# cgisky1980/Qwen3-TTS-Rust

Measured on AMD Instinct MI355X. Metric: audio_sec_per_s, higher is better.
Workload: dtype bf16

## Files before the change

include/q3tts.h:

```cpp
#ifndef Q3TTS_H
#define Q3TTS_H

#include <stdint.h>

#ifdef __cplusplus
extern "C" {
#endif

#define Q3TTS_OK 0
#define Q3TTS_ERR_INVALID (-1)
#define Q3TTS_ERR_DEVICE (-2)
#define Q3TTS_ERR_OOM (-3)
#define Q3TTS_ERR_IO (-4)
#define Q3TTS_ERR_STATE (-5)
#define Q3TTS_ERR_UNSUPPORTED (-6)
#define Q3TTS_MAX_BATCH 256

#define Q3TTS_MAX_UPSAMPLE 4
#define Q3TTS_MAX_DEC_BLOCKS 8


typedef struct q3tts_model_config {
    int32_t t_n_layer, t_d_model, t_n_head, t_n_kv_head, t_head_dim, t_d_ffn, t_vocab;
    float t_rope_theta;
// ... 272 lines not shown
                    int32_t* n_samples_out);
int q3tts_k_vocoder_latent(q3tts_engine* e, const int32_t* codes, int32_t n_frames, int32_t chunk_frames, float* out);
typedef struct q3tts_voc_tap {
    char name[32];
    int32_t dtype, layout, hist_rows, rows, channels, reserved;
    uint64_t offset;
} q3tts_voc_tap;
int q3tts_k_vocoder_taps(q3tts_engine* e, const int32_t* codes, int32_t n_frames, int32_t chunk_frames, int32_t tap_call, void* buf,
                         uint64_t buf_bytes, q3tts_voc_tap* recs, int32_t rec_cap, int32_t* n_recs);
int q3tts_k_vocoder_bench(q3tts_engine* e, int32_t n_slots, int32_t chunks, float* ms_per_chunk);
int q3tts_k_gguf_read(const char* path, const char* tensor, float* out, int64_t cap, int64_t* nelem, int64_t* dims4, int32_t* ggml_type);
int q3tts_k_gguf_meta(const char* path, const char* key, int32_t* value_type, int32_t* elem_type, int64_t* count, double* values,
                      int64_t values_cap, char* str, int64_t str_cap, int64_t* str_bytes);
int q3tts_k_probe(q3tts_engine* e, int32_t enable);
int q3tts_k_mfma_bf16(int32_t device, const uint16_t* a, const uint16_t* b, const float* c, float* d, int32_t n_cases, int32_t chain);
int q3tts_k_bgemm(int32_t device, const uint16_t* xb, int32_t B, int32_t K, const uint16_t* w_bf16, int32_t N, const float* ssp, int32_t ntiles,
                  int32_t d_norm, float eps, int32_t epilogue, const float* nw_next, float* y, uint16_t* yb, float* ssp_out, uint64_t* keys,
                  int32_t iters, float* mean_kernel_ms);
int q3tts_k_bgemm_policy(int32_t big);
int q3tts_k_attend_policy(int32_t decode, int32_t prefill);
int q3tts_k_pred_variant(q3tts_engine* e, int32_t force);
int q3tts_k_text_ready(int32_t n_text, int32_t closed, int32_t n_frames);
int q3tts_k_bgemm_pick(int32_t B, int32_t K, int32_t N, int32_t epilogue, int32_t w_once, int32_t q8, int32_t* out5);
int q3tts_k_bgemm_q8(int32_t device, const uint16_t* xb, int32_t B, int32_t K, const int8_t* q, const uint16_t* d_f16, int32_t N, const float* ssp,
                     int32_t ntiles, int32_t d_norm, float eps, int32_t epilogue, const float* nw_next, float* y, uint16_t* yb, float* ssp_out,
                     uint64_t* keys, int32_t iters, float* mean_kernel_ms);
int q3tts_k_bgemm_q8a8(int32_t device, const int8_t* aq, const float* ad, int32_t B, int32_t K, const int8_t* q, const uint16_t* d_f16, int32_t N,
                       const float* ssp, int32_t ntiles, int32_t d_norm, float eps, int32_t epilogue, const float* nw_next, float* y, int8_t* yq,
                       float* yd, float* ssp_out, int32_t iters, float* mean_kernel_ms);
int q3tts_k_bgemm_q8a8_argmax(int32_t device, const int8_t* aq, const float* ad, int32_t B, int32_t K, const int8_t* q, const uint16_t* d_f16, int32_t N,
                              const float* ssp, int32_t ntiles, int32_t d_norm, float eps, int32_t* ids_out);
int q3tts_k_bgemm_voc(int32_t device, const uint16_t* xb, int32_t B, int32_t K, const uint16_t* w_bf16, int32_t N, int32_t epilogue, const float* bias,
                      int32_t bias_n, const float* col_scale, int32_t seg_rows, int32_t gap_rows, float* y, uint16_t* yb, int32_t want_yb);
int q3tts_k_project(int32_t device, const float* x, int32_t rows, int32_t n_in, const float* w, const float* bias, int32_t n_out, const float* nw,
                    float* y, uint16_t* xb, float* ssp);
int q3tts_k_norm_inputs(int32_t device, const float* x, int32_t rows, int32_t d, const float* nw, uint16_t* xb, float* ssp);
int q3tts_k_alloc_upload(q3tts_engine* e, int64_t bytes, int64_t* mismatches);
int q3tts_k_pcm_pack(int32_t device, const float* src, int32_t rows, int64_t stride, const int32_t* ent_row, const int32_t* ent_first,
                     const int32_t* ent_count, const int64_t* ent_dst, int32_t n_ent, int32_t format, void* out, int64_t out_n);
int q3tts_k_resample_table(int32_t rate_in, int32_t rate_out, int32_t* L, int32_t* M, int32_t* H, float* tab, int64_t cap, int64_t* n);
int q3tts_k_pcm_resample(int32_t device, const float* src, int32_t rows, int64_t stride, const int32_t* row_len, const int32_t* row_final,
                         const int32_t* ent_row, const int32_t* ent_first, const int32_t* ent_count, const int64_t* ent_dst, int32_t n_ent,
                         int32_t rate_in, int32_t rate_out, int32_t format, void* out, int64_t out_n, int32_t iters, float* mean_ms);
int q3tts_k_row_buckets(int32_t max_batch, int32_t* out, int32_t cap);
int q3tts_k_bucket_steps(const q3tts_engine* e, int64_t* out, int32_t cap);
int q3tts_k_prefix_stats(const q3tts_engine* e, int64_t* out2);
// ... 9 lines not shown
```

qwen3-tts-rust_amd/csrc/q3_attend.hip:

```cpp
#include "q3_kernels.h"

__device__ __forceinline__ uint2 pack_bf16x4(float a, float b, float c, float d) {
    return make_uint2((uint32_t)q3_bf16(a) | ((uint32_t)q3_bf16(b) << 16), (uint32_t)q3_bf16(c) | ((uint32_t)q3_bf16(d) << 16));
}
__device__ __forceinline__ uint16_t* k_cache_elem(uint16_t* khead, int pos, int lane) {
    const int blk = pos >> 6, kl = pos & 63, c = lane >> 1, e0 = 4 * (lane & 1);
    return khead + ((size_t)(blk * (Q3_ATT_HD >> 3) + c) * 64 + kl) * 8 + e0;
}
__device__ __forceinline__ float prep_rinv(const float4 x4, float eps, int hd) {
    float acc = 0.0f;
    acc = fmaf(x4.x, x4.x, acc); acc = fmaf(x4.y, x4.y, acc); acc = fmaf(x4.z, x4.z, acc); acc = fmaf(x4.w, x4.w, acc);
    acc = wave_sum(acc);
    return 1.0f / sqrtf(acc / (float)hd + eps);
}
__device__ __forceinline__ void prep_norm(const float4 x4, float rinv, const float4 w4, float y[4]) {
    y[0] = (x4.x * rinv) * w4.x; y[1] = (x4.y * rinv) * w4.y; y[2] = (x4.z * rinv) * w4.z; y[3] = (x4.w * rinv) * w4.w;
}
__device__ __forceinline__ void prep_rope(const float y[4], const float4 c4, const float4 s4, int hl, int lane, float o[4]) {
    const float cc[4] = {c4.x, c4.y, c4.z, c4.w}, ss[4] = {s4.x, s4.y, s4.z, s4.w};
#pragma unroll
    for (int e = 0; e < 4; ++e) {
        const float other = __shfl_xor(y[e], hl);
        o[e] = (lane < hl) ? fmaf(-other, ss[e], y[e] * cc[e])
                           : fmaf(other, ss[e], y[e] * cc[e]);
// ... 190 lines not shown
    for (int e = 0; e < 8; ++e) {
        o[e] = o[e] + __shfl_xor(o[e], 16);
        o[e] = o[e] + __shfl_xor(o[e], 32);
    }
    if (kg == 0) {
#pragma unroll
        for (int e = 0; e < 8; ++e) ow[(hh * 4 + sw) * hd + dl * 8 + e] = o[e];
    }
    __syncthreads();
    Q3_STAMP(a, 3);
    for (int i = tid; i < R * hd; i += R * 256) {
        const int h2 = i / hd, d = i - h2 * hd;
        const float r0 = ow[(h2 * 4 + 0) * hd + d], r1 = ow[(h2 * 4 + 1) * hd + d], r2 = ow[(h2 * 4 + 2) * hd + d],
                    r3 = ow[(h2 * 4 + 3) * hd + d];
        const float ov = ((r0 + r1) + r2) + r3;
        const float l = ((lw[h2 * 4] + lw[h2 * 4 + 1]) + lw[h2 * 4 + 2]) + lw[h2 * 4 + 3];
        att_out1(a, row, g * R + h2, d, ov / l);
    }
#ifdef Q3_STAMPS
    Q3_STAMP(a, 4);
    asm volatile("s_waitcnt vmcnt(0)" ::: "memory");
    Q3_STAMP(a, 5);
#endif
}
__global__ __launch_bounds__(256, 2) void k_attend_gqa2(Q3Attend a) {
    extern __shared__ __attribute__((aligned(16))) float smem[];
    const int g = blockIdx.x, row = blockIdx.y;
    Q3_STAMP(a, 0);
    int pos, slot;
    q3_row_map(row, a.row_pos, a.row_slot, a.slot_mod, a.pos_const, &pos, &slot);
    if (pos < 0) return;
    constexpr int hd = Q3_ATT_HD, half = hd >> 1, nl = hd >> 2;
    const int T = pos + 1, Tcap = a.n_ctx;
    const int tid = threadIdx.x, sw = tid >> 6, lane = tid & 63, kg = lane >> 4, dl = lane & 15;
    float* p0 = smem;
    float* p1 = p0 + Tcap;
    float* qh = p1 + Tcap;
    float* ow = qh + 2 * hd;
    float* lw = ow + 2 * 4 * hd;
    float* mw = lw + 8;
    uint32_t* knew = (uint32_t*)(mw + 8);
    uint32_t* vnew = knew + 64;
    const Q3QkPrep& pr = a.prep;
    const size_t hb = ((size_t)slot * a.Hkv + g) * a.n_ctx;
    const uint16_t* kb = a.kc + hb * hd;
    const uint16_t* vb = a.vc + hb * hd;
// ... 14 lines not shown
            prep_norm(x4, prep_rinv(x4, pr.eps, hd), w4, y);
            const float cc[4] = {c4.x, c4.y, c4.z, c4.w}, ss[4] = {s4.x, s4.y, s4.z, s4.w};
            float o[4];
#pragma unroll
            for (int e = 0; e < 4; ++e) {
                const float other = __shfl_xor(y[e], 16);
                o[e] = (lane < 16) ? fmaf(-other, ss[e], y[e] * cc[e]) : fmaf(other, ss[e], y[e] * cc[e]);
            }
            if (lane < nl) {
                if (sw < 2) *(float4*)(qh + sw * hd + 4 * lane) = (float4){o[0], o[1], o[2], o[3]};
                else {
                    const uint2 kk = pack_bf16x4(o[0], o[1], o[2], o[3]);
                    *(uint2*)k_cache_elem(pr.kc + hb * hd, pos, lane) = kk;
                    *(uint2*)(knew + 2 * lane) = kk;
                }
            }
        } else if (lane < nl) {
            const uint2 vk = pack_bf16x4(x4.x, x4.y, x4.z, x4.w);
            *(uint2*)(pr.vc + (hb + pos) * hd + 4 * lane) = vk;
            *(uint2*)(vnew + 2 * lane) = vk;
        }
    }
    __builtin_amdgcn_sched_barrier(0);
    uint4 kv[16], vv[4][4];
    {
        const uint4* kp = (const uint4*)(kb + (size_t)min(sw, (T - 1) >> 6) * 64 * hd) + lane;
#pragma unroll
        for (int c = 0; c < 16; ++c) kv[c] = kp[c * 64];
#pragma unroll
        for (int tr = 0; tr < 2; ++tr)
#pragma unroll
            for (int u = 0; u < 4; ++u) vv[tr][u] = *(const uint4*)(vb + (size_t)min(64 * tr + 4 * sw + kg + 16 * u, T - 1) * hd + dl * 8);
    }
    __builtin_amdgcn_sched_barrier(0);
    Q3_LDS_BARRIER();
    Q3_STAMP(a, 1);
    const float scale = 1.0f / sqrtf((float)hd);
    float ml0 = -INFINITY, ml1 = -INFINITY;
    for (int blk = sw; blk * 64 < T; blk += 4) {
        const int t = blk * 64 + lane;
        if (blk != sw) {
            const uint4* kp = (const uint4*)(kb + (size_t)blk * 64 * hd) + lane;
#pragma unroll
            for (int c = 0; c < 16; ++c) kv[c] = kp[c * 64];
        }
        if (t == pos) {
#pragma unroll
            for (int c = 0; c < 16; ++c) kv[c] = *(const uint4*)(knew + 4 * c);
        }
        float s0 = 0.0f, s1 = 0.0f;
#pragma unroll
        for (int c = 0; c < 16; ++c) {
            const float4 qa = *(const float4*)(qh + c * 8), qb = *(const float4*)(qh + c * 8 + 4);
            const float4 ra = *(const float4*)(qh + hd + c * 8), rb = *(const float4*)(qh + hd + c * 8 + 4);
            s0 = att_dot8(qa, qb, kv[c], s0);
            s1 = att_dot8(ra, rb, kv[c], s1);
        }
        s0 = s0 * scale; s1 = s1 * scale;
        if (t < T) { p0[t] = s0; p1[t] = s1; ml0 = fmaxf(ml0, s0); ml1 = fmaxf(ml1, s1); }
    }
#pragma unroll
    for (int tr = 2; tr < 4; ++tr)
#pragma unroll
        for (int u = 0; u < 4; ++u) vv[tr][u] = *(const uint4*)(vb + (size_t)min(64 * tr + 4 * sw + kg + 16 * u, T - 1) * hd + dl * 8);
    ml0 = wave_max(ml0); ml1 = wave_max(ml1);
    if (lane == 0) { mw[sw] = ml0; mw[4 + sw] = ml1; }
    Q3_LDS_BARRIER();
    const float m0 = fmaxf(fmaxf(mw[0], mw[1]), fmaxf(mw[2], mw[3])), m1 = fmaxf(fmaxf(mw[4], mw[5]), fmaxf(mw[6], mw[7]));
    float ls0 = 0.0f, ls1 = 0.0f;
    for (int blk = sw; blk * 64 < T; blk += 4) {
        const int t = blk * 64 + lane;
        if (t < T) {
            const float e0 = q3_expf(p0[t] - m0), e1 = q3_expf(p1[t] - m1);
            p0[t] = e0; p1[t] = e1; ls0 += e0; ls1 += e1;
        }
    }
    ls0 = wave_sum(ls0); ls1 = wave_sum(ls1);
    if (lane == 0) { lw[sw] = ls0; lw[4 + sw] = ls1; }
    Q3_LDS_BARRIER();
    Q3_STAMP(a, 2);
    float o0[8], o1[8];
#pragma unroll
    for (int e = 0; e < 8; ++e) { o0[e] = 0.0f; o1[e] = 0.0f; }
    const uint4 vn = *(const uint4*)(vnew + 4 * dl);
#pragma unroll
    for (int tr = 0; tr < 4; ++tr) {
        const int t0 = 64 * tr + 4 * sw + kg;
        if (64 * tr >= T) break;
#pragma unroll
        for (int u = 0; u < 4; ++u) {
            const int t = t0 + 16 * u;
            if (t < T) {
                const float pa = p0[t], pb = p1[t];
                const uint4 w = (t == pos) ? vn : vv[tr][u];
                att_pv8x2(pa, pb, w, o0, o1);
            }
        }
    }
    for (int t0 = 256 + 4 * sw + kg; t0 < T; t0 += 64) {
        uint4 vl[4];
#pragma unroll
        for (int u = 0; u < 4; ++u) vl[u] = *(const uint4*)(vb + (size_t)min(t0 + 16 * u, T - 1) * hd + dl * 8);
#pragma unroll
        for (int u = 0; u < 4; ++u) {
            const int t = t0 + 16 * u;
            if (t < T) {
                const float pa = p0[t], pb = p1[t];
                const uint4 w = (t == pos) ? vn : vl[u];
                att_pv8x2(pa, pb, w, o0, o1);
            }
        }
    }
#pragma unroll
    for (int e = 0; e < 8; ++e) {
        o0[e] = o0[e] + __shfl_xor(o0[e], 16); o0[e] = o0[e] + __shfl_xor(o0[e], 32);
        o1[e] = o1[e] + __shfl_xor(o1[e], 16); o1[e] = o1[e] + __shfl_xor(o1[e], 32);
    }
    if (kg == 0) {
        *(float4*)(ow + (0 * 4 + sw) * hd + dl * 8) = (float4){o0[0], o0[1], o0[2], o0[3]}; *(float4*)(ow + (0 * 4 + sw) * hd + dl * 8 + 4) = (float4){o0[4], o0[5], o0[6], o0[7]};
        *(float4*)(ow + (1 * 4 + sw) * hd + dl * 8) = (float4){o1[0], o1[1], o1[2], o1[3]}; *(float4*)(ow + (1 * 4 + sw) * hd + dl * 8 + 4) = (float4){o1[4], o1[5], o1[6], o1[7]};
    }
    Q3_LDS_BARRIER();
    Q3_STAMP(a, 3);
    if (tid < 128) {
        const int h2 = tid >> 6, d0 = 2 * (tid & 63);
// ... 465 lines not shown
```

qwen3-tts-rust_amd/csrc/q3_bgemm.hip:

```cpp
#include "q3_kernels.h"

typedef __bf16 bf16x8 __attribute__((ext_vector_type(8)));
typedef uint32_t u32x4 __attribute__((ext_vector_type(4)));

__device__ __forceinline__ float bg_wave_sum(float v) {
#pragma unroll
    for (int m = 32; m >= 1; m >>= 1) v = v + __shfl_xor(v, m);
    return v;
}

__device__ __forceinline__ size_t bg_yoff(const Q3BGemm& g, int row) {
    return g.seg_rows ? (size_t)(row / g.seg_rows) * g.seg_stride + (size_t)(row % g.seg_rows) * g.ldy : (size_t)row * g.ldy;
}
__device__ __forceinline__ float bg_gelu_erf(float x) { return 0.5f * x * (1.0f + erff(x * 0.70710678118654752f)); }

__device__ __forceinline__ u32x4 bg_ldw(const u32x4* p, bool nt) { return nt ? __builtin_nontemporal_load(p) : *p; }

__device__ __forceinline__ bf16x8 bg_q8_frag(uint32_t lo, uint32_t hi) {
    union { u32x4 u; bf16x8 v; } r;
#define Q8F(w_, b_) __float_as_uint((float)(int)(signed char)((w_) >> (8 * (b_))))
    r.u.x = (Q8F(lo, 0) >> 16) | (Q8F(lo, 1) & 0xffff0000u); r.u.y = (Q8F(lo, 2) >> 16) | (Q8F(lo, 3) & 0xffff0000u);
    r.u.z = (Q8F(hi, 0) >> 16) | (Q8F(hi, 1) & 0xffff0000u); r.u.w = (Q8F(hi, 2) >> 16) | (Q8F(hi, 3) & 0xffff0000u);
#undef Q8F
    return r.v;
}
__device__ __forceinline__ float bg_f16(uint32_t bits) { return (float)__builtin_bit_cast(_Float16, (unsigned short)bits); }

#define BG_PH(RT_, NT_) ((8 * (RT_) * (NT_) > 64 && ((RT_) * (NT_)) % 2 == 0) ? 2 : 1)
template <int RT, int NT, int D, bool NTW, bool Q8>
__global__ __launch_bounds__(512) void k_bgemm(Q3BGemm g) {
    extern __shared__ float part[];
    __shared__ float srow[64];
    Q3_STAMP(g, 0);
    constexpr int TR = RT * NT * 4;
    const int wave = threadIdx.x >> 6, lane = threadIdx.x & 63, kq = lane >> 4, r = lane & 15;
    int cg = blockIdx.x, rc = blockIdx.y;
    if (gridDim.y > 1 && (gridDim.x & 7) == 0) {
        const int id = blockIdx.x + gridDim.x * blockIdx.y, G = gridDim.y;
        rc = (id >> 3) % G; cg = (id & 7) + (id / (8 * G)) * 8;
    }
    const int nb0 = cg * NT, row0 = rc * RT * 16, kblocks = g.K >> 5, per = g.K >> 8, kb0 = wave * per;
    const int B = g.B;
    const u32x4* ap[RT];
#pragma unroll
    for (int i = 0; i < RT; ++i) {
        const int R = g.a_row0 + min(row0 + 16 * i + r, B - 1);
        ap[i] = (const u32x4*)g.a + ((size_t)(R >> 4) * kblocks + kb0) * 64 + kq * 16 + (R & 15);
    }
    const u32x4* wp[NT];
#pragma unroll
    for (int j = 0; j < NT; ++j) wp[j] = (const u32x4*)g.w + ((size_t)(nb0 + j) * kblocks + kb0) * 64 + lane;
    constexpr int NR = 2 * RT;
// ... 374 lines not shown
                    if (g.nw_next) {
                        if (live) g.yb[q3_atile_off(row, col, g.N >> 5)] = q3_bf16(xv * g.nw_next[col]);
                        float sq = xv * xv;
                        sq = sq + __shfl_xor(sq, 1); sq = sq + __shfl_xor(sq, 2); sq = sq + __shfl_xor(sq, 4); sq = sq + __shfl_xor(sq, 8);
                        if (live && c == 0) g.ssp_out[(size_t)row * g.ld_ssp_out + tile] = sq;
                    }
                }
            }
        }
}
static bool bg_big_ok(const Q3BGemm& g) {
    return g.B >= 256 && !g.wscale && (g.epi == Q3_EPI_STORE || g.epi == Q3_EPI_RESID || g.epi == Q3_EPI_SWIGLU) && g.N % 128 == 0 && g.a_row0 % 16 == 0 &&
           !g.bias && !g.col_scale && !g.seg_rows && !(g.epi == Q3_EPI_RESID && g.yb && !g.nw_next);
}
static void bg_launch_big(const Q3BGemm& g, hipStream_t s) {
    const dim3 grid(g.N / 128, (g.B + 127) / 128);
    hipLaunchKernelGGL(k_bgemm_big, grid, dim3(256), BB_NS * 16384, s, g);
}

template <int RT, int NT>
struct BgInst {
    static constexpr int S = RT + NT;
    static constexpr int D = S <= 3 ? 8 : (S == 4 ? 5 : (S == 5 ? 4 : (S == 6 ? 3 : 2)));
    static constexpr size_t lds = (size_t)8 * RT * NT * 4 * 64 * 4 / BG_PH(RT, NT);
    static void prepare() {
        if (lds > 65536) {
            hipFuncSetAttribute((const void*)k_bgemm<RT, NT, D, false, false>, hipFuncAttributeMaxDynamicSharedMemorySize, (int)lds);
            hipFuncSetAttribute((const void*)k_bgemm<RT, NT, D, true, false>, hipFuncAttributeMaxDynamicSharedMemorySize, (int)lds);
            hipFuncSetAttribute((const void*)k_bgemm<RT, NT, D, false, true>, hipFuncAttributeMaxDynamicSharedMemorySize, (int)lds);
            hipFuncSetAttribute((const void*)k_bgemm<RT, NT, D, true, true>, hipFuncAttributeMaxDynamicSharedMemorySize, (int)lds);
        }
    }
    static void launch(const Q3BGemm& g, dim3 grid, hipStream_t s) {
        const bool nt = g.w_once && grid.y == 1;
        if (g.wscale) {
            if (nt) hipLaunchKernelGGL((k_bgemm<RT, NT, D, true, true>), grid, dim3(512), lds, s, g);
            else hipLaunchKernelGGL((k_bgemm<RT, NT, D, false, true>), grid, dim3(512), lds, s, g);
        } else if (nt) hipLaunchKernelGGL((k_bgemm<RT, NT, D, true, false>), grid, dim3(512), lds, s, g);
        else hipLaunchKernelGGL((k_bgemm<RT, NT, D, false, false>), grid, dim3(512), lds, s, g);
    }
};
#define BG_EACH(X) X(1, 1) X(1, 2) X(1, 3) X(2, 1) X(2, 2) X(2, 3) X(3, 1) X(3, 2) X(3, 3) X(4, 1) X(4, 2) X(4, 3)
static int g_lds_cap_kb = 0;
static int g_big_policy = 0;
void q3_bgemm_prepare() {
    static Q3PerDevice pd;
    static std::once_flag env_once;
    std::call_once(env_once, []() {
        const char* ev = getenv("Q3TTS_BG_BIG"); g_big_policy = ev ? atoi(ev) : 0;
        ev = getenv("Q3TTS_BG_LDS_CAP"); g_lds_cap_kb = ev ? atoi(ev) : 0;
    });
    pd.ensure(1, []() {
        hipFuncSetAttribute((const void*)k_bgemm_big, hipFuncAttributeMaxDynamicSharedMemorySize, BB_NS * 16384);
#define P(RT_, NT_) BgInst<RT_, NT_>::prepare();
        BG_EACH(P)
#undef P
    });
}

static int g_force_rt = 0, g_force_nt = 0;
void q3_bgemm_force(int rt, int nt) { g_force_rt = rt; g_force_nt = nt; }
void q3_bgemm_big_policy(int policy) { q3_bgemm_prepare(); g_big_policy = policy; }
// ... 14 lines not shown
            const bool mid = g.B > 64 && g.B <= 512 && !g.wscale;
            if (g.B > 64 && !mid && RT != 4 && !(RT == 2 && g.B <= 128)) continue;
            const long chunks = (g.B + 16 * RT - 1) / (16 * RT);
            if (g.B <= 64 && RT > 1 && 16 * (RT - 1) * chunks >= g.B) continue;
            const long wgs = (long)(tiles / NT) * chunks, rounds = (wgs + 255) / 256;
            const long cost = rounds * ((g.wscale ? 32L * RT + 17L * NT : 32L * (RT + NT)) * g.K + 24000L);
            const bool tie = mid ? (NT > bestNT || (NT == bestNT && wgs > bestWgs)) : (wgs > bestWgs || (wgs == bestWgs && NT > bestNT));
            if (bestCost < 0 || cost < bestCost || (cost == bestCost && tie)) { bestCost = cost; bestRT = RT; bestNT = NT; bestWgs = wgs; }
        }
    if (g_force_rt > 0 && g_force_nt > 0 && tiles % g_force_nt == 0) { bestRT = g_force_rt; bestNT = g_force_nt; }
    *rt = bestRT; *nt = bestNT;
}
void q3_bgemm_pick(const Q3BGemm& g, int* rt, int* nt, int* d, int* ntw, int* big) {
    q3_bgemm_prepare();
    bg_pick(g, rt, nt, big);
    *d = 0; *ntw = 0;
    if (*big) return;
#define X(RT_, NT_) if (*rt == RT_ && *nt == NT_) *d = BgInst<RT_, NT_>::D;
    BG_EACH(X)
#undef X
    *ntw = (g.w_once && (g.B + 16 * *rt - 1) / (16 * *rt) == 1) ? 1 : 0;
}

static int bg_check(const Q3BGemm& g) {
    if (g.B < 1 || g.N % 16 || g.K % 256 || g.K < 256 || !g.a || !g.w || g.a_row0 < 0) return -1;
    if (g.wscale && g.K % 512) return -1;
    if (g.yb && (((g.epi == Q3_EPI_RESID || g.epi == Q3_EPI_GELU) && g.N % 32) || (g.epi == Q3_EPI_SWIGLU && g.N % 64))) return -1;
    if ((g.epi == Q3_EPI_SWIGLU || g.epi == Q3_EPI_GELU) && (!g.yb)) return -1;
    if (g.bias && g.bias_n < 1) return -1;
    if (g.ssp && g.ntiles < 1) return -1;
    return 0;
}

int q3_launch_bgemm(const Q3BGemm& g, hipStream_t s) {
    if (bg_check(g)) return -1;
    q3_bgemm_prepare();
    int bestRT, bestNT, big;
    bg_pick(g, &bestRT, &bestNT, &big);
    if (big) { bg_launch_big(g, s); return 0; }
    const dim3 grid(g.N / 16 / bestNT, (g.B + 16 * bestRT - 1) / (16 * bestRT));
#define L(RT_, NT_) if (bestRT == RT_ && bestNT == NT_) { BgInst<RT_, NT_>::launch(g, grid, s); return 0; }
    BG_EACH(L)
#undef L
    return -1;
}

// ... 22 lines not shown
```

qwen3-tts-rust_amd/csrc/q3_hooks.hip:

```cpp
#include "q3_engine.h"

#include <cstdio>
#include <cstring>

#define TRY(x) do { int rc__ = (x); if (rc__ != Q3TTS_OK) return rc__; } while (0)
#define HK(call) do { hipError_t er__ = (call); if (er__ != hipSuccess) return q3_set_err(nullptr, Q3TTS_ERR_DEVICE, std::string(#call) + ": " + hipGetErrorString(er__)); } while (0)

struct DevBuf {
    void* p = nullptr;
    ~DevBuf() { if (p) hipFree(p); }
    template <class T> operator T*() const { return (T*)p; }
    int put(const void* host, size_t bytes) {
        if (hipMalloc(&p, bytes + 64) != hipSuccess || hipMemset(p, 0, bytes + 64) != hipSuccess) return q3_set_err(nullptr, Q3TTS_ERR_OOM, "hipMalloc");
        if (host) HK(hipMemcpy(p, host, bytes, hipMemcpyHostToDevice));
        return Q3TTS_OK;
    }
    int alloc(size_t bytes) { return put(nullptr, bytes); }
    int get(void* host, size_t bytes) const { HK(hipMemcpy(host, p, bytes, hipMemcpyDeviceToHost)); return Q3TTS_OK; }
};

template <class F>
static int time_launches(int iters, F launch, float* mean_ms) {
    if (iters <= 0 || !mean_ms) return Q3TTS_OK;
    hipEvent_t a, b; HK(hipEventCreate(&a)); HK(hipEventCreate(&b));
// ... 151 lines not shown
    qp.cs = dcs; qp.sn = dsn; qp.kc = dkc; qp.vc = dvc; qp.n_ctx = n_ctx; qp.row_pos = dpp; qp.row_slot = dps;
    if (npre && q3_launch_qk_prep(qp, nullptr)) return q3_set_err(nullptr, Q3TTS_ERR_INVALID, "attention decode hook: the q/k prep launch was refused");
    int old_dec = 0, old_pre = 0;
    q3_attend_policy_get(&old_dec, &old_pre);
    if (policy >= 0) q3_attend_policy(policy, old_pre);
    for (int pass = 0; pass < (out_bf16 ? 2 : 1); ++pass) {
        HK(hipMemcpy(dlast.p, last.data(), last.size() * 4, hipMemcpyHostToDevice));
        Q3QkPrep dq = qp; dq.qkv = dlast; dq.rows = n_slots; dq.row_pos = ddp; dq.row_slot = dds;
        Q3Attend at{}; at.qkv = dlast; at.ld = ld; at.rows = n_slots; at.ldo = nq; at.Hq = Hq; at.Hkv = Hkv; at.hd = hd;
        at.kc = dkc; at.vc = dvc; at.n_ctx = n_ctx; at.row_pos = dq.row_pos; at.row_slot = dq.row_slot;
        at.fused = 1; at.prep = dq;
        if (pass == 0) { at.out = dout; at.out_bf16 = 0; }
        else { at.out = dob; at.out_bf16 = 1; }
        if (q3_launch_attend(at, nullptr)) { q3_attend_policy(old_dec, old_pre); return q3_set_err(nullptr, Q3TTS_ERR_INVALID, "attention decode hook: the attention launch was refused"); }
        const hipError_t er = hipDeviceSynchronize();
        if (er != hipSuccess) { q3_attend_policy(old_dec, old_pre); return q3_set_err(nullptr, Q3TTS_ERR_DEVICE, std::string("attention decode hook: ") + hipGetErrorString(er)); }
    }
    q3_attend_policy(old_dec, old_pre);
    HK(hipGetLastError());
    TRY(dout.get(out_f32, (size_t)n_slots * nq * 4));
    return out_bf16 ? untile_host(dob, n_slots, nq, out_bf16) : Q3TTS_OK;
}

struct AttHook {
    int n_slots = 0, n_ctx = 0, Hq = 0, Hkv = 0, ld = 0, nq = 0, form = 0, out_rows = 0, rt16 = 0;
    DevBuf qn, kn, cs, sn, kc, vc, out, osc;
    static const char* check(const float* qkv, int n_slots, int n_ctx, int Hq, int Hkv, int hd, const float* qnw, const float* knw, int form, const void* out,
                             const float* out_scale) {
        if (!qkv || !qnw || !knw || !out) return "a null argument";
        if (hd != Q3_ATT_HD) return "head_dim must be 128";
        if (n_slots <= 0 || n_slots > 4096) return "1 .. 4096 slots";
        if (n_ctx <= 0 || n_ctx % 64 || n_ctx > 8192) return "n_ctx must be a multiple of 64 in 64 .. 8192";
        if (Hkv <= 0 || Hq <= 0 || Hq % Hkv || Hq > 64) return "n_head must be a multiple of n_kv_head";
        const int R = Hq / Hkv;
        if (R != 1 && R != 2 && R != 4) return "the GQA ratio must be 1, 2 or 4";
        if (form < 0 || form > 2) return "out_form 0 (f32), 1 (bf16) or 2 (Q8_0)";
        if (form == 2 && !out_scale) return "out_form 2 needs out_scale";
        return nullptr;
    }
    int init(int slots, int nctx, int hq, int hkv, const float* qnw, const float* knw, float theta, const int32_t* sections, int out_form, int rows) {
        n_slots = slots; n_ctx = nctx; Hq = hq; Hkv = hkv; ld = (hq + 2 * hkv) * Q3_ATT_HD; nq = hq * Q3_ATT_HD; form = out_form; out_rows = rows;
        rt16 = (int)(pad16(rows) / 16);
        std::vector<float> c, s;
        q3_rope_tables(n_ctx, Q3_ATT_HD, theta, sections, c, s);
        TRY(qn.put(qnw, Q3_ATT_HD * 4)); TRY(kn.put(knw, Q3_ATT_HD * 4)); TRY(cs.put(c.data(), c.size() * 4)); TRY(sn.put(s.data(), s.size() * 4));
        const size_t cache = (size_t)n_slots * Hkv * n_ctx * Q3_ATT_HD * 2;
        TRY(kc.alloc(cache)); TRY(vc.alloc(cache));
        TRY(out.alloc(form == 0 ? (size_t)rows * nq * 4 : pad16(rows) * nq * (form == 1 ? 2 : 1)));
        if (form == 2) TRY(osc.alloc((size_t)(nq / 32 + 2) * pad16(rows) * 4));
        return Q3TTS_OK;
    }
    Q3QkPrep prep(float* rows_dev, int rows, float eps) const {
        Q3QkPrep qp{}; qp.qkv = rows_dev; qp.ld = ld; qp.rows = rows; qp.Hq = Hq; qp.Hkv = Hkv; qp.hd = Q3_ATT_HD; qp.qnw = qn; qp.knw = kn; qp.eps = eps;
        qp.cs = cs; qp.sn = sn; qp.kc = kc; qp.vc = vc; qp.n_ctx = n_ctx;
        return qp;
    }
    Q3Attend attend(const float* rows_dev, int rows) const {
        Q3Attend at{}; at.qkv = rows_dev; at.ld = ld; at.rows = rows; at.out = out; at.ldo = nq; at.out_bf16 = form; at.Hq = Hq; at.Hkv = Hkv; at.hd = Q3_ATT_HD;
        at.kc = kc; at.vc = vc; at.n_ctx = n_ctx;
        if (form == 2) { at.out_scale = osc; at.out_rt16 = rt16; }
        return at;
    }
    int read_out(void* host, float* host_scale) const {
        if (form == 0) return out.get(host, (size_t)out_rows * nq * 4);
        if (form == 1) return untile_host(out, out_rows, nq, (uint16_t*)host);
        const size_t B16 = pad16(out_rows);
        std::vector<int8_t> qt(B16 * nq); std::vector<float> st((size_t)(nq / 32) * B16);
        TRY(out.get(qt.data(), qt.size())); TRY(osc.get(st.data(), st.size() * 4));
        for (int r = 0; r < out_rows; ++r) {
            for (int k = 0; k < nq; ++k) ((int8_t*)host)[(size_t)r * nq + k] = qt[q3_q8_off(r, k, nq >> 6)];
// ... 542 lines not shown
    if (er == hipSuccess) er = hipDeviceSynchronize();
    if (er == hipSuccess) er = hipMemcpy(back.data(), q, 8192, hipMemcpyDeviceToHost);
    if (er == hipSuccess) er = hipMemcpy(back.data() + 8192, (char*)q + bytes - 4096, 4096, hipMemcpyDeviceToHost);
    hipFree(q);
    if (er != hipSuccess) return q3_set_err(e, Q3TTS_ERR_DEVICE, hipGetErrorString(er));
    int64_t bad = 0;
    for (int i = 0; i < 4096; ++i) bad += (back[i] != pat[i]) + (back[4096 + i] != 0) + (back[8192 + i] != pat[i]);
    *mismatches = bad;
    return Q3TTS_OK;
}

extern "C" int q3tts_k_bgemm_policy(int32_t big) {
    if (big < -1 || big > 1) return q3_set_err(nullptr, Q3TTS_ERR_INVALID, "bgemm policy: -1, 0 or 1");
    q3_bgemm_big_policy(big);
    return Q3TTS_OK;
}

extern "C" int q3tts_k_attend_policy(int32_t decode, int32_t prefill) {
    if (decode < 0 || decode > 1 || prefill < 0 || prefill > 2) return q3_set_err(nullptr, Q3TTS_ERR_INVALID, "attend policy: decode 0..1, prefill 0..2");
    q3_attend_policy(decode, prefill);
    return Q3TTS_OK;
}

extern "C" int q3tts_k_pred_variant(q3tts_engine* e, int32_t force) {
    if (!e) return q3_set_err(nullptr, Q3TTS_ERR_INVALID, "null engine");
    Q3_NOT_IN_SESSION(e);
    if (force < 0 || force > 1) return q3_set_err(e, Q3TTS_ERR_INVALID, "pred variant: 0 or 1");
    return q3_pred_force_variant(e, force);
}

extern "C" int q3tts_k_bgemm_pick(int32_t B, int32_t K, int32_t N, int32_t epilogue, int32_t w_once, int32_t q8, int32_t* out5) {
    if (!out5 || B < 1 || K < 256 || K % 256 || N % 16) return q3_set_err(nullptr, Q3TTS_ERR_INVALID, "bgemm pick: bad shape");
    Q3BGemm g{}; g.B = B; g.K = K; g.N = N; g.epi = epilogue; g.w_once = w_once;
    g.a = (const uint16_t*)16; g.w = (const uint4*)16; g.wscale = q8 ? (const uint16_t*)16 : nullptr;
    if (epilogue == Q3_EPI_SWIGLU || epilogue == Q3_EPI_GELU) g.yb = (uint16_t*)16;
    if (epilogue == Q3_EPI_RESID) { g.yb = (uint16_t*)16; g.nw_next = (const float*)16; }
    int rt, nt, d, ntw, big;
    q3_bgemm_pick(g, &rt, &nt, &d, &ntw, &big);
    out5[0] = rt; out5[1] = nt; out5[2] = d; out5[3] = ntw; out5[4] = big;
    return Q3TTS_OK;
}

extern "C" int q3tts_k_pcm_pack(int32_t device, const float* src, int32_t rows, int64_t stride, const int32_t* ent_row, const int32_t* ent_first,
                                const int32_t* ent_count, const int64_t* ent_dst, int32_t n_ent, int32_t format, void* out, int64_t out_n) {
    if (!src || !out || rows <= 0 || stride <= 0 || stride > (1 << 28) || n_ent < 0 || n_ent > Q3_PCM_MAX_ENT || (format != 0 && format != 1) || out_n < 0 ||
        (n_ent > 0 && (!ent_row || !ent_first || !ent_count || !ent_dst)))
        return q3_set_err(nullptr, Q3TTS_ERR_INVALID, "pcm pack hook: bad arguments");
    Q3PcmPack pk{};
    int mx = 0;
    for (int j = 0; j < n_ent; ++j) {
        const long long r = ent_row[j], f = ent_first[j], c = ent_count[j], d = ent_dst[j];
        if (r < 0 || r >= rows || f < 0 || c < 0 || f + c > stride || d < 0 || d + c > out_n)
            return q3_set_err(nullptr, Q3TTS_ERR_INVALID, "pcm pack hook: a window lies outside src or out");
        pk.e[j] = Q3PcmEnt{(int32_t)r, (int32_t)f, (int32_t)c, 0, d};
        mx = std::max(mx, (int)c);
    }
    const size_t es = format ? 2 : 4;
    HK(hipSetDevice(device));
    DevBuf s, o;
    TRY(s.put(src, sizeof(float) * (size_t)rows * stride)); TRY(o.alloc(es * (size_t)std::max<int64_t>(out_n, 1)));
    if (out_n > 0) HK(hipMemcpy(o.p, out, es * (size_t)out_n, hipMemcpyHostToDevice));
    q3_launch_pcm_pack(s, (size_t)stride, pk, n_ent, mx, format, o.p, nullptr);
// ... 65 lines not shown
```

qwen3-tts-rust_amd/csrc/q3_kernels.h:

```cpp
#pragma once
#include "q3_common.h"

enum { Q3_EPI_STORE = 0, Q3_EPI_RESID = 1, Q3_EPI_SWIGLU = 2, Q3_EPI_ARGMAX = 3, Q3_EPI_GELU = 4 };

#ifdef Q3_STAMPS
#define Q3_STAMP_FIELD unsigned long long* dbg;
#define Q3_STAMP(p, i) do { if ((p).dbg && threadIdx.x == 0) (p).dbg[((size_t)blockIdx.x + (size_t)gridDim.x * blockIdx.y) * 8 + (i)] = __builtin_amdgcn_s_memrealtime(); } while (0)
#else
#define Q3_STAMP_FIELD
#define Q3_STAMP(p, i) do { } while (0)
#endif

#include <mutex>
#include <type_traits>
#include <vector>
struct Q3PerDevice {
    std::mutex mu; size_t have[64] = {0};
    template <class F> bool ensure(size_t want, F set_attr) {
        int dev = 0; if (hipGetDevice(&dev) != hipSuccess) dev = 0;
        std::lock_guard<std::mutex> lk(mu);
        if (have[dev & 63] >= want) return true;
        if constexpr (std::is_void_v<decltype(set_attr())>) set_attr();
        else if (set_attr() != hipSuccess) return false;
        have[dev & 63] = want;
// ... 31 lines not shown
}
struct Q3BGemm {
    const uint16_t* a; int a_row0; int B;
    const uint4* w; int K, N;
    int w_once;
    const float* ssp; int ld_ssp; int ntiles; int d_norm; float eps;
    int epi;
    float* y; int ldy;
    uint16_t* yb;
    const float* nw_next; float* ssp_out; int ld_ssp_out;
    const float* col_scale;
    const float* bias; int bias_n;
    int seg_rows; size_t seg_stride;
    unsigned long long* keys; int key_stride;
    const uint16_t* wscale;
    const float* ascale; int a_rt16; float* yscale; int y_rt16;
    Q3_STAMP_FIELD
};
int q3_launch_bgemm(const Q3BGemm& g, hipStream_t s);
int q3_launch_bgemm8(const Q3BGemm& g, hipStream_t s);
void q3_bgemm8_prepare();
void q3_bgemm8_pick(const Q3BGemm& g, int* rt, int* nt);
void q3_bgemm_pick(const Q3BGemm& g, int* rt, int* nt, int* d, int* ntw, int* big);
void q3_bgemm_force(int rt, int nt);
void q3_bgemm_prepare();
void q3_bgemm_big_policy(int policy);
void q3_launch_norm_inputs(const float* x, int ldx, int rows, int d, const float* nw, uint16_t* xb, int xb_row0, float* ssp, int ld_ssp, hipStream_t s);
void q3_launch_norm_inputs_q8(const float* x, int ldx, int rows, int d, const float* nw, int8_t* xq, float* xscale, int rt16, float* ssp, int ld_ssp, hipStream_t s);
struct Q3Project {
    const float* x; int ldx; int rows;
    const float* w; const float* bias; int n_in, n_out;
    float* y; int ldy;
    const float* nw; uint16_t* xb; float* ssp; int ld_ssp;
    const float* norm_w; float eps;
    float* xscale; int x_rt16;
};
int q3_launch_project(const Q3Project& p, hipStream_t s);
#define Q3_LDS_BARRIER() do { asm volatile("s_waitcnt lgkmcnt(0)" ::: "memory"); __builtin_amdgcn_s_barrier(); asm volatile("" ::: "memory"); } while (0)
#ifdef __HIPCC__
__device__ __forceinline__ float wave_sum(float v) {
#pragma unroll
    for (int m = 32; m >= 1; m >>= 1) v = v + __shfl_xor(v, m);
    return v;
}
__device__ __forceinline__ float wave_max(float v) {
#pragma unroll
// ... 196 lines not shown
```

qwen3-tts-rust_amd/q3tts/_abi.py:

```python
import ctypes as C
import os

HERE = os.path.dirname(os.path.abspath(__file__))
PKG_ROOT = os.path.dirname(HERE)
REPO_ROOT = os.path.dirname(PKG_ROOT)
LIB_PATH = os.path.join(PKG_ROOT, "csrc", "libq3tts.so")

Q3TTS_MAX_UPSAMPLE = 4
Q3TTS_MAX_DEC_BLOCKS = 8


class ModelConfig(C.Structure):
    _fields_ = [
        ("t_n_layer", C.c_int32), ("t_d_model", C.c_int32), ("t_n_head", C.c_int32), ("t_n_kv_head", C.c_int32),
        ("t_head_dim", C.c_int32), ("t_d_ffn", C.c_int32), ("t_vocab", C.c_int32),
        ("t_rope_theta", C.c_float),
        ("t_mrope_sections", C.c_int32 * 4),
        ("p_n_layer", C.c_int32), ("p_d_model", C.c_int32), ("p_n_head", C.c_int32), ("p_n_kv_head", C.c_int32),
        ("p_head_dim", C.c_int32), ("p_d_ffn", C.c_int32),
        ("p_rope_theta", C.c_float),
        ("n_codebooks", C.c_int32), ("codebook_size", C.c_int32),
        ("rms_eps", C.c_float),
        ("d_embed", C.c_int32), ("text_vocab", C.c_int32), ("codec0_rows", C.c_int32), ("codecq_rows", C.c_int32),
        ("sample_limit", C.c_int32), ("eos_code", C.c_int32), ("tts_pad_id", C.c_int32),
# ... 104 lines not shown
        ("ae_d_ffn", C.c_int32), ("ae_window", C.c_int32),
        ("ae_rope_theta", C.c_float), ("ae_ln_eps", C.c_float), ("ae_layer_scale", C.c_float),
        ("ae_down_stride", C.c_int32), ("ae_vq_dim", C.c_int32), ("ae_n_codebooks", C.c_int32), ("ae_codebook_size", C.c_int32),
    ]


SYMBOLS = [
    "q3tts_default_config", "q3tts_engine_create", "q3tts_engine_destroy", "q3tts_last_error", "q3tts_set_sampler",
    "q3tts_set_max_steps", "q3tts_build_prompt", "q3tts_free", "q3tts_generate", "q3tts_generate_batch",
    "q3tts_result_free", "q3tts_stream_begin", "q3tts_stream_poll", "q3tts_stream_end",
    "q3tts_get_timings", "q3tts_k_gemm_exact", "q3tts_k_attention", "q3tts_k_attention_decode", "q3tts_k_sample", "q3tts_k_talker_prefill",
    "q3tts_k_vocoder", "q3tts_k_vocoder_latent", "q3tts_k_vocoder_taps", "q3tts_k_vocoder_bench", "q3tts_set_device_pcm", "q3tts_get_device_pcm", "q3tts_k_rng_f32", "q3tts_k_probe", "q3tts_k_gguf_read", "q3tts_mel_frames", "q3tts_mel",
    "q3tts_clone_default_config", "q3tts_clone_init", "q3tts_clone_audio_frames", "q3tts_clone_audio_encode",
    "q3tts_clone_speaker_encode", "q3tts_k_speaker_from_mel", "q3tts_k_audio_latent",
    "q3tts_node_create", "q3tts_node_destroy", "q3tts_node_generate_batch", "q3tts_node_get_timings", "q3tts_node_last_error", "q3tts_node_size", "q3tts_node_engine", "q3tts_node_shard", "q3tts_k_bgemm_q8", "q3tts_k_bgemm_q8a8_argmax", "q3tts_k_bgemm_q8a8", "q3tts_k_alloc_upload", "q3tts_k_bgemm_policy", "q3tts_k_attend_policy", "q3tts_k_bgemm_pick", "q3tts_k_mfma_bf16", "q3tts_k_bgemm", "q3tts_k_bgemm_voc", "q3tts_k_project", "q3tts_k_norm_inputs", "q3tts_tokenizer_load", "q3tts_tokenizer_free", "q3tts_tokenizer_vocab_size", "q3tts_tokenizer_encode", "q3tts_tokenizer_decode",
    "q3tts_session_create", "q3tts_session_submit", "q3tts_session_cancel", "q3tts_session_next", "q3tts_session_close",
    "q3tts_session_last_error", "q3tts_k_pcm_pack",
    "q3tts_prefix_create", "q3tts_prefix_rows", "q3tts_prefix_destroy", "q3tts_k_talker_prefill_prefix",
    "q3tts_config_from_model_dir", "q3tts_k_gguf_meta",
    "q3tts_set_predictor_sampler", "q3tts_get_predictor_sampler", "q3tts_set_repetition_penalty", "q3tts_get_repetition_penalty",
    "q3tts_k_pred_variant",
    "q3tts_set_output_rate", "q3tts_get_output_rate", "q3tts_resample", "q3tts_k_resample_table", "q3tts_k_pcm_resample",
    "q3tts_session_append_text", "q3tts_k_text_ready",
    "q3tts_k_attention_runs", "q3tts_k_attention_decode_ex", "q3tts_k_attention_pair", "q3tts_k_attend_pick",
    "q3tts_k_pred_table_row", "q3tts_k_pred_next", "q3tts_k_attention_gather",
    "q3tts_k_row_buckets", "q3tts_k_bucket_steps", "q3tts_k_device_bytes", "q3tts_k_engine_footprint", "q3tts_k_prefix_stats",
]


class PredStep(C.Structure):
    _fields_ = [
        ("n_rows", C.c_int32), ("q", C.c_int32), ("n_codebooks", C.c_int32), ("n_key_parts", C.c_int32), ("rows_q", C.c_int32),
        ("d_embed", C.c_int32), ("d_proj", C.c_int32), ("max_steps_cap", C.c_int32),
        ("keys", C.c_void_p), ("active", C.c_void_p), ("n_frames", C.c_void_p), ("codec_q", C.c_void_p), ("pproj_q", C.c_void_p),
        ("proj_b", C.c_void_p), ("fb", C.c_void_p), ("px", C.c_void_p), ("codes", C.c_void_p),
    ]


class Q3Error(RuntimeError):
    pass


_lib = None


def load_library(path=None):
    global _lib
# ... 106 lines not shown
    lib.q3tts_k_bgemm_voc.argtypes = [C.c_int32, C.c_void_p, C.c_int32, C.c_int32, C.c_void_p, C.c_int32, C.c_int32, C.c_void_p, C.c_int32, C.c_void_p,
                                      C.c_int32, C.c_int32, C.c_void_p, C.c_void_p, C.c_int32]
    lib.q3tts_node_create.argtypes = [C.POINTER(EngineConfig), i32p, C.c_int32, C.POINTER(vp)]
    lib.q3tts_node_destroy.argtypes = [vp]
    lib.q3tts_node_destroy.restype = None
    lib.q3tts_node_generate_batch.argtypes = [vp, C.POINTER(Request), C.c_int32, C.POINTER(Result), C.POINTER(C.POINTER(C.c_int16))]
    lib.q3tts_node_get_timings.argtypes = [vp, C.POINTER(NodeTimings)]
    lib.q3tts_node_last_error.argtypes = [vp]
    lib.q3tts_node_last_error.restype = C.c_char_p
    lib.q3tts_node_size.argtypes = [vp]
    lib.q3tts_node_size.restype = C.c_int32
    lib.q3tts_node_engine.argtypes = [vp, C.c_int32]
    lib.q3tts_node_engine.restype = vp
    lib.q3tts_node_shard.argtypes = [C.c_int32, C.c_int32, C.c_int32, i32p, C.c_int32]
    lib.q3tts_node_shard.restype = C.c_int32
    lib.q3tts_k_bgemm_q8.argtypes = [C.c_int32, C.c_void_p, C.c_int32, C.c_int32, C.c_void_p, C.c_void_p, C.c_int32, C.c_void_p, C.c_int32, C.c_int32, C.c_float,
                                     C.c_int32, C.c_void_p, C.c_void_p, C.c_void_p, C.c_void_p, C.c_void_p, C.c_int32, f32p]
    lib.q3tts_k_bgemm_q8a8_argmax.argtypes = [C.c_int32, C.c_void_p, C.c_void_p, C.c_int32, C.c_int32, C.c_void_p, C.c_void_p, C.c_int32, C.c_void_p, C.c_int32, C.c_int32, C.c_float, C.c_void_p]
    lib.q3tts_k_bgemm_q8a8_argmax.restype = C.c_int
    lib.q3tts_k_bgemm_q8a8.argtypes = [C.c_int32, C.c_void_p, C.c_void_p, C.c_int32, C.c_int32, C.c_void_p, C.c_void_p, C.c_int32, C.c_void_p, C.c_int32, C.c_int32, C.c_float,
                                       C.c_int32, C.c_void_p, C.c_void_p, C.c_void_p, C.c_void_p, C.c_void_p, C.c_int32, f32p]
    lib.q3tts_k_bgemm_policy.argtypes = [C.c_int32]
    lib.q3tts_k_attend_policy.argtypes = [C.c_int32, C.c_int32]
    lib.q3tts_k_bgemm_pick.argtypes = [C.c_int32, C.c_int32, C.c_int32, C.c_int32, C.c_int32, C.c_int32, i32p]
    lib.q3tts_k_alloc_upload.argtypes = [vp, C.c_int64, C.POINTER(C.c_int64)]
    lib.q3tts_k_row_buckets.argtypes = [C.c_int32, i32p, C.c_int32]
    lib.q3tts_k_bucket_steps.argtypes = [vp, C.POINTER(C.c_int64), C.c_int32]
    lib.q3tts_k_device_bytes.argtypes = [vp, C.POINTER(C.c_int64)]
    lib.q3tts_k_prefix_stats.argtypes = [vp, C.POINTER(C.c_int64)]
    lib.q3tts_k_engine_footprint.argtypes = [C.POINTER(EngineConfig), C.POINTER(C.c_int64)]
    lib.q3tts_tokenizer_load.argtypes = [C.c_char_p, C.POINTER(vp), C.c_char_p, C.c_int32]
    lib.q3tts_tokenizer_free.argtypes = [vp]
    lib.q3tts_tokenizer_free.restype = None
    lib.q3tts_tokenizer_vocab_size.argtypes = [vp]
    lib.q3tts_tokenizer_vocab_size.restype = C.c_int32
    lib.q3tts_tokenizer_encode.argtypes = [vp, C.c_char_p, C.c_int64, u32p, C.c_int32, i32p, C.c_char_p, C.c_int32]
    lib.q3tts_tokenizer_decode.argtypes = [vp, u32p, C.c_int32, C.c_char_p, C.c_int64, C.POINTER(C.c_int64), C.c_char_p, C.c_int32]
    if path is None:
        _lib = lib
    return lib


def default_config():
    cfg = EngineConfig()
    load_library().q3tts_default_config(C.byref(cfg))
    return cfg
# ... 101 lines not shown
```

Baseline: 685.0.

## Use buffer loads with OOB masking in attention and cap bgemm ring depth by K

Attention K/V loads now go through raw buffer resources, so out-of-range rows return zero via hardware bounds checks instead of clamped redundant reads of row T-1. The bgemm kernel gains a ring-depth template parameter, chosen at launch from K/256, so short-K GEMMs use a shallower pipeline ring. The intent is to avoid wasted memory traffic in attention tails and over-deep prefetch rings for small K, at the cost of more kernel instantiations. Test hooks for cache fill patterns and forcing bgemm tiles are also added.

```diff
diff --git a/include/q3tts.h b/include/q3tts.h
--- a/include/q3tts.h
+++ b/include/q3tts.h
@@ -318,6 +318,9 @@
 int q3tts_k_pred_variant(q3tts_engine* e, int32_t force);
 int q3tts_k_text_ready(int32_t n_text, int32_t closed, int32_t n_frames);
 int q3tts_k_bgemm_pick(int32_t B, int32_t K, int32_t N, int32_t epilogue, int32_t w_once, int32_t q8, int32_t* out5);
+int q3tts_k_bgemm_pick_ex(int32_t B, int32_t K, int32_t N, int32_t epilogue, int32_t w_once, int32_t q8, int32_t* out6);
+int q3tts_k_bgemm_force(int32_t rt, int32_t nt);
+int q3tts_k_attend_cache_fill(int32_t bf16_bits);
 int q3tts_k_bgemm_q8(int32_t device, const uint16_t* xb, int32_t B, int32_t K, const int8_t* q, const uint16_t* d_f16, int32_t N, const float* ssp,
                      int32_t ntiles, int32_t d_norm, float eps, int32_t epilogue, const float* nw_next, float* y, uint16_t* yb, float* ssp_out,
                      uint64_t* keys, int32_t iters, float* mean_kernel_ms);
diff --git a/qwen3-tts-rust_amd/csrc/q3_attend.hip b/qwen3-tts-rust_amd/csrc/q3_attend.hip
--- a/qwen3-tts-rust_amd/csrc/q3_attend.hip
+++ b/qwen3-tts-rust_amd/csrc/q3_attend.hip
@@ -236,6 +236,14 @@
     asm volatile("s_waitcnt vmcnt(0)" ::: "memory");
     Q3_STAMP(a, 5);
 #endif
+}
+#define ATT_OOB 0x80000000u
+__device__ __forceinline__ __amdgpu_buffer_rsrc_t att_rsrc(const uint16_t* base, uint32_t bytes) {
+    return __builtin_amdgcn_make_buffer_rsrc((void*)base, 0, (int)bytes, 0x00020000);
+}
+__device__ __forceinline__ uint4 att_ldb16(__amdgpu_buffer_rsrc_t rs, uint32_t off) {
+    const auto v = __builtin_amdgcn_raw_buffer_load_b128(rs, (int)off, 0, 0);
+    return make_uint4(v[0], v[1], v[2], v[3]);
 }
 __global__ __launch_bounds__(256, 2) void k_attend_gqa2(Q3Attend a) {
     extern __shared__ __attribute__((aligned(16))) float smem[];
@@ -296,15 +304,17 @@
         }
     }
     __builtin_amdgcn_sched_barrier(0);
+    const __amdgpu_buffer_rsrc_t krs = att_rsrc(kb, (uint32_t)a.n_ctx * hd * 2), vrs = att_rsrc(vb, (uint32_t)T * hd * 2);
+    const uint32_t voff = (uint32_t)(4 * sw + kg) * hd * 2 + dl * 16;
     uint4 kv[16], vv[4][4];
     {
-        const uint4* kp = (const uint4*)(kb + (size_t)min(sw, (T - 1) >> 6) * 64 * hd) + lane;
-#pragma unroll
-        for (int c = 0; c < 16; ++c) kv[c] = kp[c * 64];
+        const uint32_t koff = sw * 64 + lane < T ? (uint32_t)(sw * 64 * hd + lane * 8) * 2 : ATT_OOB;
+#pragma unroll
+        for (int c = 0; c < 16; ++c) kv[c] = att_ldb16(krs, koff + c * 1024);
 #pragma unroll
         for (int tr = 0; tr < 2; ++tr)
 #pragma unroll
-            for (int u = 0; u < 4; ++u) vv[tr][u] = *(const uint4*)(vb + (size_t)min(64 * tr + 4 * sw + kg + 16 * u, T - 1) * hd + dl * 8);
+            for (int u = 0; u < 4; ++u) vv[tr][u] = att_ldb16(vrs, voff + (64 * tr + 16 * u) * hd * 2);
     }
     __builtin_amdgcn_sched_barrier(0);
     Q3_LDS_BARRIER();
@@ -314,9 +324,9 @@
     for (int blk = sw; blk * 64 < T; blk += 4) {
         const int t = blk * 64 + lane;
         if (blk != sw) {
-            const uint4* kp = (const uint4*)(kb + (size_t)blk * 64 * hd) + lane;
-#pragma unroll
-            for (int c = 0; c < 16; ++c) kv[c] = kp[c * 64];
+            const uint32_t koff = t < T ? (uint32_t)(blk * 64 * hd + lane * 8) * 2 : ATT_OOB;
+#pragma unroll
+            for (int c = 0; c < 16; ++c) kv[c] = att_ldb16(krs, koff + c * 1024);
         }
         if (t == pos) {
 #pragma unroll
@@ -336,7 +346,7 @@
 #pragma unroll
     for (int tr = 2; tr < 4; ++tr)
 #pragma unroll
-        for (int u = 0; u < 4; ++u) vv[tr][u] = *(const uint4*)(vb + (size_t)min(64 * tr + 4 * sw + kg + 16 * u, T - 1) * hd + dl * 8);
+        for (int u = 0; u < 4; ++u) vv[tr][u] = att_ldb16(vrs, voff + (64 * tr + 16 * u) * hd * 2);
     ml0 = wave_max(ml0); ml1 = wave_max(ml1);
     if (lane == 0) { mw[sw] = ml0; mw[4 + sw] = ml1; }
     Q3_LDS_BARRIER();
@@ -374,7 +384,7 @@
     for (int t0 = 256 + 4 * sw + kg; t0 < T; t0 += 64) {
         uint4 vl[4];
 #pragma unroll
-        for (int u = 0; u < 4; ++u) vl[u] = *(const uint4*)(vb + (size_t)min(t0 + 16 * u, T - 1) * hd + dl * 8);
+        for (int u = 0; u < 4; ++u) vl[u] = att_ldb16(vrs, (uint32_t)(t0 + 16 * u) * hd * 2 + dl * 16);
 #pragma unroll
         for (int u = 0; u < 4; ++u) {
             const int t = t0 + 16 * u;
diff --git a/qwen3-tts-rust_amd/csrc/q3_bgemm.hip b/qwen3-tts-rust_amd/csrc/q3_bgemm.hip
--- a/qwen3-tts-rust_amd/csrc/q3_bgemm.hip
+++ b/qwen3-tts-rust_amd/csrc/q3_bgemm.hip
@@ -27,7 +27,8 @@
 __device__ __forceinline__ float bg_f16(uint32_t bits) { return (float)__builtin_bit_cast(_Float16, (unsigned short)bits); }
 
 #define BG_PH(RT_, NT_) ((8 * (RT_) * (NT_) > 64 && ((RT_) * (NT_)) % 2 == 0) ? 2 : 1)
-template <int RT, int NT, int D, bool NTW, bool Q8>
+static constexpr int bg_ring_depth(int D, int per) { return per >= D ? D : (per >= 4 ? (D > 4 ? 4 : D) : (D > 2 ? 2 : D)); }
+template <int RT, int NT, int DI, bool NTW, bool Q8, int D>
 __global__ __launch_bounds__(512) void k_bgemm(Q3BGemm g) {
     extern __shared__ float part[];
     __shared__ float srow[64];
@@ -448,22 +449,36 @@
 struct BgInst {
     static constexpr int S = RT + NT;
     static constexpr int D = S <= 3 ? 8 : (S == 4 ? 5 : (S == 5 ? 4 : (S == 6 ? 3 : 2)));
+    static constexpr int D4 = D > 4 ? 4 : D, D2 = D > 2 ? 2 : D;
     static constexpr size_t lds = (size_t)8 * RT * NT * 4 * 64 * 4 / BG_PH(RT, NT);
+    template <int DD>
+    static void prepare_d() {
+        hipFuncSetAttribute((const void*)k_bgemm<RT, NT, D, false, false, DD>, hipFuncAttributeMaxDynamicSharedMemorySize, (int)lds);
+        hipFuncSetAttribute((const void*)k_bgemm<RT, NT, D, true, false, DD>, hipFuncAttributeMaxDynamicSharedMemorySize, (int)lds);
+        hipFuncSetAttribute((const void*)k_bgemm<RT, NT, D, false, true, DD>, hipFuncAttributeMaxDynamicSharedMemorySize, (int)lds);
+        hipFuncSetAttribute((const void*)k_bgemm<RT, NT, D, true, true, DD>, hipFuncAttributeMaxDynamicSharedMemorySize, (int)lds);
+    }
     static void prepare() {
         if (lds > 65536) {
-            hipFuncSetAttribute((const void*)k_bgemm<RT, NT, D, false, false>, hipFuncAttributeMaxDynamicSharedMemorySize, (int)lds);
-            hipFuncSetAttribute((const void*)k_bgemm<RT, NT, D, true, false>, hipFuncAttributeMaxDynamicSharedMemorySize, (int)lds);
-            hipFuncSetAttribute((const void*)k_bgemm<RT, NT, D, false, true>, hipFuncAttributeMaxDynamicSharedMemorySize, (int)lds);
-            hipFuncSetAttribute((const void*)k_bgemm<RT, NT, D, true, true>, hipFuncAttributeMaxDynamicSharedMemorySize, (int)lds);
-        }
-    }
-    static void launch(const Q3BGemm& g, dim3 grid, hipStream_t s) {
+            prepare_d<D>();
+            if (D4 != D) prepare_d<D4>();
+            if (D2 != D4) prepare_d<D2>();
+        }
+    }
+    template <int DD>
+    static void launch_d(const Q3BGemm& g, dim3 grid, hipStream_t s) {
         const bool nt = g.w_once && grid.y == 1;
         if (g.wscale) {
-            if (nt) hipLaunchKernelGGL((k_bgemm<RT, NT, D, true, true>), grid, dim3(512), lds, s, g);
-            else hipLaunchKernelGGL((k_bgemm<RT, NT, D, false, true>), grid, dim3(512), lds, s, g);
-        } else if (nt) hipLaunchKernelGGL((k_bgemm<RT, NT, D, true, false>), grid, dim3(512), lds, s, g);
-        else hipLaunchKernelGGL((k_bgemm<RT, NT, D, false, false>), grid, dim3(512), lds, s, g);
+            if (nt) hipLaunchKernelGGL((k_bgemm<RT, NT, D, true, true, DD>), grid, dim3(512), lds, s, g);
+            else hipLaunchKernelGGL((k_bgemm<RT, NT, D, false, true, DD>), grid, dim3(512), lds, s, g);
+        } else if (nt) hipLaunchKernelGGL((k_bgemm<RT, NT, D, true, false, DD>), grid, dim3(512), lds, s, g);
+        else hipLaunchKernelGGL((k_bgemm<RT, NT, D, false, false, DD>), grid, dim3(512), lds, s, g);
+    }
+    static void launch(const Q3BGemm& g, dim3 grid, hipStream_t s) {
+        const int d = bg_ring_depth(D, g.K >> 8);
+        if (d == D) launch_d<D>(g, grid, s);
+        else if (d == D4) launch_d<D4>(g, grid, s);
+        else launch_d<D2>(g, grid, s);
     }
 };
 #define BG_EACH(X) X(1, 1) X(1, 2) X(1, 3) X(2, 1) X(2, 2) X(2, 3) X(3, 1) X(3, 2) X(3, 3) X(4, 1) X(4, 2) X(4, 3)
@@ -524,6 +539,8 @@
     *ntw = (g.w_once && (g.B + 16 * *rt - 1) / (16 * *rt) == 1) ? 1 : 0;
 }
 
+int q3_bgemm_ring_depth(int d, int K) { return bg_ring_depth(d, K >> 8); }
+
 static int bg_check(const Q3BGemm& g) {
     if (g.B < 1 || g.N % 16 || g.K % 256 || g.K < 256 || !g.a || !g.w || g.a_row0 < 0) return -1;
     if (g.wscale && g.K % 512) return -1;
diff --git a/qwen3-tts-rust_amd/csrc/q3_hooks.hip b/qwen3-tts-rust_amd/csrc/q3_hooks.hip
--- a/qwen3-tts-rust_amd/csrc/q3_hooks.hip
+++ b/qwen3-tts-rust_amd/csrc/q3_hooks.hip
@@ -197,6 +197,7 @@
     return out_bf16 ? untile_host(dob, n_slots, nq, out_bf16) : Q3TTS_OK;
 }
 
+static int g_att_cache_fill = 0;
 struct AttHook {
     int n_slots = 0, n_ctx = 0, Hq = 0, Hkv = 0, ld = 0, nq = 0, form = 0, out_rows = 0, rt16 = 0;
     DevBuf qn, kn, cs, sn, kc, vc, out, osc;
@@ -221,6 +222,7 @@
         TRY(qn.put(qnw, Q3_ATT_HD * 4)); TRY(kn.put(knw, Q3_ATT_HD * 4)); TRY(cs.put(c.data(), c.size() * 4)); TRY(sn.put(s.data(), s.size() * 4));
         const size_t cache = (size_t)n_slots * Hkv * n_ctx * Q3_ATT_HD * 2;
         TRY(kc.alloc(cache)); TRY(vc.alloc(cache));
+        if (g_att_cache_fill) { HK(hipMemsetD16(kc.p, (unsigned short)g_att_cache_fill, cache / 2)); HK(hipMemsetD16(vc.p, (unsigned short)g_att_cache_fill, cache / 2)); }
         TRY(out.alloc(form == 0 ? (size_t)rows * nq * 4 : pad16(rows) * nq * (form == 1 ? 2 : 1)));
         if (form == 2) TRY(osc.alloc((size_t)(nq / 32 + 2) * pad16(rows) * 4));
         return Q3TTS_OK;
@@ -809,6 +811,18 @@
     return Q3TTS_OK;
 }
 
+extern "C" int q3tts_k_attend_cache_fill(int32_t bf16_bits) {
+    if (bf16_bits < 0 || bf16_bits > 0xffff) return q3_set_err(nullptr, Q3TTS_ERR_INVALID, "attend cache fill: a 16-bit pattern");
+    g_att_cache_fill = bf16_bits;
+    return Q3TTS_OK;
+}
+
+extern "C" int q3tts_k_bgemm_force(int32_t rt, int32_t nt) {
+    if (!((rt == 0 && nt == 0) || (rt >= 1 && rt <= 4 && nt >= 1 && nt <= 3))) return q3_set_err(nullptr, Q3TTS_ERR_INVALID, "bgemm force: (0, 0) or row tiles 1..4, column tiles 1..3");
+    q3_bgemm_force(rt, nt);
+    return Q3TTS_OK;
+}
+
 extern "C" int q3tts_k_pred_variant(q3tts_engine* e, int32_t force) {
     if (!e) return q3_set_err(nullptr, Q3TTS_ERR_INVALID, "null engine");
     Q3_NOT_IN_SESSION(e);
@@ -825,6 +839,13 @@
     int rt, nt, d, ntw, big;
     q3_bgemm_pick(g, &rt, &nt, &d, &ntw, &big);
     out5[0] = rt; out5[1] = nt; out5[2] = d; out5[3] = ntw; out5[4] = big;
+    return Q3TTS_OK;
+}
+
+extern "C" int q3tts_k_bgemm_pick_ex(int32_t B, int32_t K, int32_t N, int32_t epilogue, int32_t w_once, int32_t q8, int32_t* out6) {
+    if (!out6) return q3_set_err(nullptr, Q3TTS_ERR_INVALID, "bgemm pick: bad shape");
+    if (const int rc = q3tts_k_bgemm_pick(B, K, N, epilogue, w_once, q8, out6)) return rc;
+    out6[5] = out6[4] ? 0 : q3_bgemm_ring_depth(out6[2], K);
     return Q3TTS_OK;
 }
 
diff --git a/qwen3-tts-rust_amd/csrc/q3_kernels.h b/qwen3-tts-rust_amd/csrc/q3_kernels.h
--- a/qwen3-tts-rust_amd/csrc/q3_kernels.h
+++ b/qwen3-tts-rust_amd/csrc/q3_kernels.h
@@ -77,6 +77,7 @@
 void q3_bgemm8_prepare();
 void q3_bgemm8_pick(const Q3BGemm& g, int* rt, int* nt);
 void q3_bgemm_pick(const Q3BGemm& g, int* rt, int* nt, int* d, int* ntw, int* big);
+int q3_bgemm_ring_depth(int d, int K);
 void q3_bgemm_force(int rt, int nt);
 void q3_bgemm_prepare();
 void q3_bgemm_big_policy(int policy);
diff --git a/qwen3-tts-rust_amd/q3tts/_abi.py b/qwen3-tts-rust_amd/q3tts/_abi.py
--- a/qwen3-tts-rust_amd/q3tts/_abi.py
+++ b/qwen3-tts-rust_amd/q3tts/_abi.py
@@ -150,7 +150,7 @@
     "q3tts_k_pred_variant",
     "q3tts_set_output_rate", "q3tts_get_output_rate", "q3tts_resample", "q3tts_k_resample_table", "q3tts_k_pcm_resample",
     "q3tts_session_append_text", "q3tts_k_text_ready",
-    "q3tts_k_attention_runs", "q3tts_k_attention_decode_ex", "q3tts_k_attention_pair", "q3tts_k_attend_pick",
+    "q3tts_k_attention_runs", "q3tts_k_attention_decode_ex", "q3tts_k_attention_pair", "q3tts_k_attend_pick", "q3tts_k_attend_cache_fill", "q3tts_k_bgemm_force", "q3tts_k_bgemm_pick_ex",
     "q3tts_k_pred_table_row", "q3tts_k_pred_next", "q3tts_k_attention_gather",
     "q3tts_k_row_buckets", "q3tts_k_bucket_steps", "q3tts_k_device_bytes", "q3tts_k_engine_footprint", "q3tts_k_prefix_stats",
 ]
@@ -303,6 +303,9 @@
                                        C.c_int32, C.c_void_p, C.c_void_p, C.c_void_p, C.c_void_p, C.c_void_p, C.c_int32, f32p]
     lib.q3tts_k_bgemm_policy.argtypes = [C.c_int32]
     lib.q3tts_k_attend_policy.argtypes = [C.c_int32, C.c_int32]
+    lib.q3tts_k_attend_cache_fill.argtypes = [C.c_int32]
+    lib.q3tts_k_bgemm_force.argtypes = [C.c_int32, C.c_int32]
+    lib.q3tts_k_bgemm_pick_ex.argtypes = [C.c_int32, C.c_int32, C.c_int32, C.c_int32, C.c_int32, C.c_int32, i32p]
     lib.q3tts_k_bgemm_pick.argtypes = [C.c_int32, C.c_int32, C.c_int32, C.c_int32, C.c_int32, C.c_int32, i32p]
     lib.q3tts_k_alloc_upload.argtypes = [vp, C.c_int64, C.POINTER(C.c_int64)]
     lib.q3tts_k_row_buckets.argtypes = [C.c_int32, i32p, C.c_int32]
```

Result: no change. 701.3 (median of 5 runs) (+2.4%).
